# elador/FeatureDetection

Hardware: AMD Instinct MI355X
Metric: Mpatches/s (extract+WVM+SVM) per GPU, 640x480 pyramid (higher is better)
Workload: dtype u8/i32/f32/f64; 1 GPU; config 1/metric config: ffpDetectApp FaceFrontal.cfg five-stage cascade on 640x480 BGR frames: 13-layer pyramid, 20x20 windows step 1 (16185 windows/frame), HistEq64 -> WVM 280 filters -> OE -> RBF-SVM 1024 SV -> NMS; fd_pyramid_update_frames + fd_detect_five_stage_frames (the frames of a call share one pyramid aren...; frames_per_call=64, calls_in_flight=11, parallelism=image-shard dp1

## Files before the change

### featuredetection_amd/csrc/pyramid.hip

```cpp
#include "fd_internal.hpp"
#include <algorithm>
#include <cstring>

namespace {

constexpr int MAXJ = 16;

struct ResizeJob {
    int dw, dh;
    uint32_t dst_off;
    double scale_x, scale_y;
};
struct ResizeJobs {
    int n;
    ResizeJob j[MAXJ];
};
struct DownJob {
    int sw, sh;
    uint32_t src_off, dst_off;
};
struct FusedJob {
    int dw0, dh0, dw1, dh1;
    uint32_t dst0_off;
    uint32_t dst1_off;
    uint32_t xtab, ytab;
};
struct FusedJobs {
    int n;
    FusedJob j[MAXJ];
};
struct DownJobs {
    int n;
    int tile0[MAXJ + 1];
    DownJob j[MAXJ];
};
struct FilterJob {
    int w, h;
    uint32_t src_off, dst_off;
};
struct FilterJobs {
    int n;
    FilterJob j[MAXJ];
};

__device__ __forceinline__ int reflect101(int p, int len) {
    if (len == 1) return 0;
    while (p < 0 || p >= len) {
        if (p < 0) p = -p;
        else p = 2 * len - 2 - p;
    }
    return p;
}
__device__ __forceinline__ int reflect1(int p, int len) {
    if (len < 3) return reflect101(p, len);
    const int q = p < 0 ? -p : (p >= len ? 2 * len - 2 - p : p);
    return min(max(q, 0), len - 1);
}

struct FramePtrs {
    const uint8_t* p[FD_MAX_FRAMES];
};
__device__ __forceinline__ unsigned int mul24(unsigned int a, unsigned int b) {
    unsigned int r;
    asm("v_mul_u32_u24 %0, %1, %2" : "=v"(r) : "v"(a), "v"(b));
    return r;
}
__device__ __forceinline__ unsigned int mul24_s(unsigned int a_uniform, unsigned int b) {
    unsigned int r;
    asm("v_mul_u32_u24 %0, %1, %2" : "=v"(r) : "s"(a_uniform), "v"(b));
    return r;
}
__device__ __forceinline__ unsigned int mad24(unsigned int a, unsigned int b, unsigned int c) {
    unsigned int r;
    asm("v_mad_u32_u24 %0, %1, %2, %3" : "=v"(r) : "v"(a), "v"(b), "v"(c));
    return r;
}
__device__ __forceinline__ unsigned int mulhi24_s(unsigned int a_uniform, unsigned int b) {
    unsigned int r;
    asm("v_mul_hi_u32_u24 %0, %1, %2" : "=v"(r) : "s"(a_uniform), "v"(b));
    return r;
}
__device__ __forceinline__ uint32_t ld_u32_unaligned(const uint8_t* p) {
    uint32_t v;
    __builtin_memcpy(&v, p, 4);
    return v;
}
__device__ __forceinline__ uint32_t gray_of(uint32_t b, uint32_t g, uint32_t r) { return (b * 1868u + g * 9617u + r * 4899u + 8192u) >> 14; }

__global__ void k_frames_to_gray(FramePtrs frames, uint8_t* __restrict__ grayBase, size_t imageStride, int n, int ch) {
    const uint8_t* __restrict__ src = frames.p[blockIdx.y];
    uint8_t* __restrict__ gray = grayBase + (size_t)blockIdx.y * imageStride;
    const int nq = n >> 2;
    const bool aligned = ((uintptr_t)src & 3) == 0;
    const int stride = gridDim.x * blockDim.x;
    auto load3 = [&](int q, uint32_t (&w)[3]) {
        if (aligned) {
            const uint32_t* s3 = reinterpret_cast<const uint32_t*>(src) + 3 * (size_t)q;
            w[0] = s3[0]; w[1] = s3[1]; w[2] = s3[2];
        } else {
            const uint8_t* s1 = src + 12 * (size_t)q;
            w[0] = ld_u32_unaligned(s1); w[1] = ld_u32_unaligned(s1 + 4); w[2] = ld_u32_unaligned(s1 + 8);
        }
    };
    auto gray4 = [&](const uint32_t (&w)[3]) {
        const uint32_t g0 = gray_of(w[0] & 255u, (w[0] >> 8) & 255u, (w[0] >> 16) & 255u);
        const uint32_t g1 = gray_of(w[0] >> 24, w[1] & 255u, (w[1] >> 8) & 255u);
        const uint32_t g2 = gray_of((w[1] >> 16) & 255u, w[1] >> 24, w[2] & 255u);
        const uint32_t g3 = gray_of((w[2] >> 8) & 255u, (w[2] >> 16) & 255u, w[2] >> 24);
        return g0 | (g1 << 8) | (g2 << 16) | (g3 << 24);
    };
    constexpr int GQ = 4;
    for (int q = blockIdx.x * blockDim.x + threadIdx.x; q < nq; q += GQ * stride) {
        if (ch == 3) {
            uint32_t w[GQ][3];
// ... 157 lines not shown
        const int dx = dx0 + c;
        if (dx < jb.dw) {
            float fx;
            const int sx = srcX(dx, fx);
            const int a0 = __float2int_rn((1.f - fx) * 2048), a1 = __float2int_rn(fx * 2048);
            const int lx = sx - X0, lx1 = (sx + 1 < sw ? sx + 1 : sx) - X0;
            uint8_t* dp = dst + (uint32_t)((dy0 + rq * (TL_H / 4)) * jb.dw) + dx;
#pragma unroll
            for (int k = 0; k < TL_H / 4; ++k, dp += jb.dw) {
                const int rr = rq * (TL_H / 4) + k;
                if (dy0 + rr < jb.dh) {
                    const int4 rt = rowTab[rr];
                    const uint8_t* S0 = tile + rt.x;
                    const uint8_t* S1 = tile + rt.y;
                    const unsigned int r0 = __umul24(S0[lx], a0) + __umul24(S0[lx1], a1);
                    const unsigned int r1 = __umul24(S1[lx], a0) + __umul24(S1[lx1], a1);
                    *dp = (uint8_t)(((__umul24(rt.z, r0 >> 4) >> 16) + (__umul24(rt.w, r1 >> 4) >> 16) + 2) >> 2);
                }
            }
        }
        __syncthreads();
    }
}

#ifdef FD_PYR_PROF
constexpr int PYR_PROF_WGS = 65536;
__device__ unsigned long long fd_pyr_prof[PYR_PROF_WGS * 8];
#define PYR_T(x) const unsigned long long x = __builtin_amdgcn_s_memtime()
#else
#define PYR_T(x)
#endif
constexpr int FT_W1 = 62, FT_H1 = 16;
constexpr int G0_W = 2 * FT_W1 + 3, G0_H = 2 * FT_H1 + 3, G0_PITCH = 128;
constexpr int FS_PITCH = 256, FS_ROWS = 76;
constexpr int FS_LOADS = (FS_ROWS + 3) / 4;
struct FusedFetch {
    uint32_t v[FS_LOADS];
    int2 ex, ey;
};
__device__ __forceinline__ void fused_issue(FusedFetch& f, const uint8_t* __restrict__ src, int sw, const int2* __restrict__ tabs, const FusedJob& jb,
                                            const int4 d) {
    const int X0 = d.x & 0xffff, Y0 = (int)((uint32_t)d.x >> 16), ncol = d.y & 0xffff, nrow = (int)((uint32_t)d.y >> 16);
    const int gx0 = 2 * (d.z & 0xffff) * FT_W1 - 2;
    const int lane = threadIdx.x & 63, wave = __builtin_amdgcn_readfirstlane(threadIdx.x >> 6);
    const uint32_t voff = (uint32_t)(4 * min(lane, (ncol - 1) >> 2) + X0);
    const int rlast = nrow - 1;
#pragma unroll
    for (int q = 0; q < FS_LOADS; ++q) {
        const int r = min(wave + 4 * q, rlast);
        f.v[q] = ld_u32_unaligned(src + (uint32_t)((Y0 + r) * sw) + voff);
    }
    f.ex = tabs[jb.xtab + reflect101(gx0 + (int)(threadIdx.x & 127), jb.dw0)];
    {
        const int py = 2 * (int)((uint32_t)d.z >> 16) * FT_H1 - 2 + min(lane, G0_H - 1), pr = py < 0 ? -py : (py >= jb.dh0 ? 2 * jb.dh0 - 2 - py : py);
        f.ey = tabs[jb.ytab + min(max(pr, 0), jb.dh0 - 1)];
    }
}

__global__ __launch_bounds__(256) void k_resize_down(uint8_t* __restrict__ arena0, uint32_t src_off, int sw, int sh, const int2* __restrict__ tabs,
                                                     FusedJobs jobs, uint32_t tileTab, int tilesPerFrame, int nimg, size_t imageStride) {
    __shared__ __attribute__((aligned(16))) uint8_t stage[FS_ROWS * FS_PITCH];
    __shared__ __attribute__((aligned(16))) uint8_t g0[G0_H * G0_PITCH];
    const int4* tiles = reinterpret_cast<const int4*>(tabs + tileTab);
    const int lane = threadIdx.x & 63, wave = __builtin_amdgcn_readfirstlane(threadIdx.x >> 6);
    const bool byXcd = nimg >= 8 && (gridDim.x & 7u) == 0;
    const int xcd = blockIdx.x & 7;
    const int slot = byXcd ? (int)(blockIdx.x >> 3) : (int)blockIdx.x, nslot = byXcd ? (int)(gridDim.x >> 3) : (int)gridDim.x;
    const int items = (byXcd ? (nimg - xcd + 7) >> 3 : nimg) * tilesPerFrame;
    auto frame_of = [&](int item) { const int fi = item / tilesPerFrame; return byXcd ? xcd + 8 * fi : fi; };
    auto desc_of = [&](int item) { return item < items ? tiles[item % tilesPerFrame] : make_int4(0, 0, 0, 0); };

    int item = slot;
    if (item >= items) return;
    int4 d = desc_of(item);
    FusedFetch f;
    fused_issue(f, arena0 + (size_t)frame_of(item) * imageStride + src_off, sw, tabs, jobs.j[d.w], d);
    int itemN = item + nslot;
    int4 dN = desc_of(itemN);

#ifdef FD_PYR_PROF
    unsigned long long pacc[6] = {0, 0, 0, 0, 0, 0}, ptiles = 0;
#endif
    for (; item < items; item = itemN, d = dN, itemN += nslot, dN = desc_of(itemN)) {
        PYR_T(p0);
        const FusedJob jb = jobs.j[d.w];
        uint8_t* arena = arena0 + (size_t)frame_of(item) * imageStride;
        const int X0 = d.x & 0xffff, Y0 = (int)((uint32_t)d.x >> 16);
        const int x1 = (d.z & 0xffff) * FT_W1, y1 = (int)((uint32_t)d.z >> 16) * FT_H1;
        const int gx0 = 2 * x1 - 2, gy0 = 2 * y1 - 2;
        {
            static_assert(4 * (FS_LOADS - 1) + 3 < FS_ROWS && FS_PITCH == 256, "stage holds a dword per lane for rows wave + 4 q");
#pragma unroll
            for (int q = 0; q < FS_LOADS; ++q) *reinterpret_cast<uint32_t*>(&stage[(wave + 4 * q) * FS_PITCH + 4 * lane]) = f.v[q];
        }
        const int2 ex = f.ex, ey = f.ey;
        PYR_T(p1);
        __syncthreads();
        PYR_T(p2);
        if (itemN < items)
            fused_issue(f, arena0 + (size_t)frame_of(itemN) * imageStride + src_off, sw, tabs, jobs.j[dN.w], dN);
        PYR_T(p3);
        {
            const int c = threadIdx.x & 127, half = __builtin_amdgcn_readfirstlane(threadIdx.x >> 7);
            if (c < G0_W) {
                const uint8_t* sp = stage + (ex.x - X0);
                const unsigned int a0 = ex.y & 0xffff, a1 = (unsigned int)ex.y >> 16;
                uint8_t* gp = g0 + c;
                const unsigned int rowRec = (unsigned int)((ey.x & 0xffff) - Y0) | (((unsigned int)ey.y & 0xfffu) << 7) | ((((unsigned int)ey.y >> 16) & 0xfffu) << 19);
                const int rBase = half * (G0_H - 18);
#pragma unroll 2
                for (int i = 0; i < 18; i += 3) {
                    unsigned int s00[3], s01[3], s10[3], s11[3], b0s[3], b1s[3];
#pragma unroll
                    for (int q = 0; q < 3; ++q) {
                        const int r = rBase + i + q;
                        const unsigned int e = (unsigned int)__builtin_amdgcn_readlane((int)rowRec, r);
                        b0s[q] = ((e >> 7) & 0xfffu) << 12;
                        b1s[q] = (e >> 19) << 12;
                        const uint8_t* sr = sp + ((e & 127u) << 8);
                        s00[q] = sr[0]; s01[q] = sr[1]; s10[q] = sr[FS_PITCH]; s11[q] = sr[FS_PITCH + 1];
                    }
#pragma unroll
                    for (int q = 0; q < 3; ++q) {
                        const unsigned int h0 = mad24(s01[q], a1, mul24(s00[q], a0)) & ~15u;
                        const unsigned int h1 = mad24(s11[q], a1, mul24(s10[q], a0)) & ~15u;
                        const unsigned int v = (mulhi24_s(b0s[q], h0) + mulhi24_s(b1s[q], h1) + 2) >> 2;
                        gp[(rBase + i + q) * G0_PITCH] = (uint8_t)v;
                    }
                }
            }
        }
        PYR_T(p4);
        __syncthreads();
        PYR_T(p5);
        {
            const int c1 = lane;
            const int x = x1 + c1;
            if (c1 < FT_W1 && x < jb.dw1) {
                constexpr int PR = FT_H1 / 4;
                const uint8_t* T = g0 + (2 * wave * PR) * G0_PITCH + 2 * c1;
                int h[2 * PR + 3];
#pragma unroll
                for (int r = 0; r < 2 * PR + 3; ++r) {
                    const uint8_t* S = T + r * G0_PITCH;
                    const uint32_t p01 = *reinterpret_cast<const uint16_t*>(S), p23 = *reinterpret_cast<const uint16_t*>(S + 2);
                    h[r] = (int)__builtin_amdgcn_udot4(p01 | (p23 << 16), 0x04060401u, (uint32_t)S[4], false);
                }
                uint8_t* dp = arena + jb.dst1_off + (uint32_t)((y1 + wave * PR) * jb.dw1) + x;
#pragma unroll
                for (int j = 0; j < PR; ++j, dp += jb.dw1) {
                    if (y1 + wave * PR + j < jb.dh1) {
                        const int v = h[2 * j + 2] * 6 + (h[2 * j + 1] + h[2 * j + 3]) * 4 + h[2 * j] + h[2 * j + 4];
                        *dp = (uint8_t)((v + 128) >> 8);
                    }
                }
            }
        }
        if (jb.dst0_off != 0xffffffffu) {
            uint8_t* d0 = arena + jb.dst0_off;
            for (int i = threadIdx.x; i < 32 * 128; i += 256) {
                const int r = 2 + (i >> 7), c = 2 + (i & 127);
// ... 60 lines not shown
                        const uint8_t* row = src + (uint32_t)(reflect_cf(Y0 + r, sh) * sw);
                        uint32_t w = 0;
#pragma unroll
                        for (int b = 0; b < 4; ++b) w |= (uint32_t)row[reflect_cf(xs + b, sw)] << (8 * b);
                        v[k] = w;
                    }
                }
            }
#pragma unroll
            for (int k = 0; k < PD_LD; ++k) *reinterpret_cast<uint32_t*>(&tile[(2 * (rq + 4 * k) + half) * TL_PITCH + j4]) = v[k];
        }
        __syncthreads();
        const int x = dx0 + c;
        if (c < PD_W && x < dw) {
            constexpr int PR = PD_TH / 4;
            const uint8_t* T = tile + (2 * rq * PR) * TL_PITCH + 2 * c;
            int h[2 * PR + 3];
#pragma unroll
            for (int r = 0; r < 2 * PR + 3; ++r) {
                const uint8_t* S = T + r * TL_PITCH;
                const uint32_t p01 = *reinterpret_cast<const uint16_t*>(S), p23 = *reinterpret_cast<const uint16_t*>(S + 2);
                h[r] = (int)__builtin_amdgcn_udot4(p01 | (p23 << 16), 0x04060401u, (uint32_t)S[4], false);
            }
            uint8_t* dp = dst + (uint32_t)((dy0 + rq * PR) * dw) + x;
#pragma unroll
            for (int j = 0; j < PR; ++j, dp += dw) {
                if (dy0 + rq * PR + j < dh) {
                    const int v = h[2 * j + 2] * 6 + (h[2 * j + 1] + h[2 * j + 3]) * 4 + h[2 * j] + h[2 * j + 4];
                    *dp = (uint8_t)((v + 128) >> 8);
                }
            }
        }
        __syncthreads();
    }
}

__device__ __forceinline__ float grad_pair(const uint8_t* __restrict__ src, int w, int h, int x, int y, int ksize, int& gx, int& gy) {
    if (ksize == 1 || ksize == 3) {
        const int xm = reflect101(x - 1, w), xp = reflect101(x + 1, w);
        const int ym = reflect101(y - 1, h), yp = reflect101(y + 1, h);
        const uint8_t *S0 = src + (size_t)ym * w, *S1 = src + (size_t)y * w, *S2 = src + (size_t)yp * w;
        if (ksize == 1) {
            gx = S1[xp] - S1[xm];
            gy = S2[x] - S0[x];
            return 0.5f;
        }
        gx = (S0[xp] - S0[xm]) + 2 * (S1[xp] - S1[xm]) + (S2[xp] - S2[xm]);
        gy = (S2[xm] - S0[xm]) + 2 * (S2[x] - S0[x]) + (S2[xp] - S0[xp]);
        return 0.125f;
    }
    int a, d1, d2, d3, s0, s1, s2, s3;
    float scale;
    if (ksize == 5) { a = 2; d1 = 2; d2 = 1; d3 = 0; s0 = 6; s1 = 4; s2 = 1; s3 = 0; scale = 1.f / 128.f; }
    else if (ksize == 7) { a = 3; d1 = 5; d2 = 4; d3 = 1; s0 = 20; s1 = 15; s2 = 6; s3 = 1; scale = 1.f / 2048.f; }
    else { a = 1; d1 = 1; d2 = 0; d3 = 0; s0 = 10; s1 = 3; s2 = 0; s3 = 0; scale = 1.f / 32.f; }
    const int dk[4] = {0, d1, d2, d3}, sk[4] = {s0, s1, s2, s3};
    int cx[7], cy[7];
    for (int t = -a; t <= a; ++t) { cx[t + a] = reflect101(x + t, w); cy[t + a] = reflect101(y + t, h); }
    gx = 0;
    gy = 0;
    for (int j = -a; j <= a; ++j) {
        const uint8_t* S = src + (size_t)cy[j + a] * w;
        int rd = 0, rs = 0;
        for (int i = 1; i <= a; ++i) {
            const int hi = S[cx[a + i]], lo = S[cx[a - i]];
            rd += dk[i] * (hi - lo);
// ... 151 lines not shown
    lut.resize((size_t)65536 * E);
    for (int x = 0; x < 256; ++x) {
        double gradientX = ((double)x - 127) / 255;
        for (int y = 0; y < 256; ++y) {
            double gradientY = ((double)y - 127) / 255;
            double direction = std::atan2(gradientY, gradientX);
            double magnitude = std::sqrt(gradientX * gradientX + gradientY * gradientY);
            double bin;
            if (signedGradients) {
                direction += PI;
                bin = direction * bins / (2 * PI);
            } else {
                if (direction < 0) direction += PI;
                bin = direction * bins / PI;
            }
            auto sat = [](double v) { int r = fd_cvRound(v); return (uint8_t)(r < 0 ? 0 : (r > 255 ? 255 : r)); };
            size_t index = (size_t)x | ((size_t)y << 8);
            if (!interpolate) {
                lut[2 * index] = (uint8_t)((uint8_t)std::round(bin) % (unsigned)bins);
                lut[2 * index + 1] = sat(255 * magnitude);
            } else {
                uint8_t w1 = sat(255 * magnitude * (bin - std::floor(bin)));
                lut[4 * index] = (uint8_t)((uint8_t)std::floor(bin) % (unsigned)bins);
                lut[4 * index + 1] = sat(255 * magnitude - w1);
                lut[4 * index + 2] = (uint8_t)((uint8_t)std::ceil(bin) % (unsigned)bins);
                lut[4 * index + 3] = w1;
            }
        }
    }
}

void build_resize_tables(fd_pyramid* p, int W, int H) {
    p->rtab_x.assign(p->all.size(), ~0u);
    p->rtab_y.assign(p->all.size(), ~0u);
    static const int mode = [] { const char* e = getenv("FD_PYR_FUSED"); return e ? atoi(e) : 1; }();
    if (mode == 0) return;
    std::vector<int2> tab;
    std::vector<std::vector<int4>> tiles;
    p->rtile_off.clear();
    p->rtile_cnt.clear();
    int nfused = 0;
    for (size_t k = 0; k + 1 < p->all.size(); ++k) {
        const HostLayer& L = p->all[k];
        const HostLayer& D = p->all[k + 1];
        if (L.depth != 0 || D.depth != 1 || D.chain != L.chain) continue;
        if (L.w == W && L.h == H && L.gray_off == p->gray_full_off) continue;
        if (L.w < 3 || L.h < 3 || W > 65535 || H > 65535) continue;
        if (L.kept && mode != 2) continue;
        const double scale_x = 1. / ((double)L.w / W), scale_y = 1. / ((double)L.h / H);
        std::vector<int2> xt((size_t)L.w), yt((size_t)L.h);
        for (int dx = 0; dx < L.w; ++dx) {
            float fx = (float)((dx + 0.5) * scale_x - 0.5);
            int sx = (int)floorf(fx);
            fx -= sx;
            if (sx < 0) { fx = 0; sx = 0; }
            if (sx >= W - 1) { fx = 0; sx = W - 1; }
            const int a0 = (int)nearbyintf((1.f - fx) * 2048), a1 = (int)nearbyintf(fx * 2048);
            xt[(size_t)dx] = make_int2(sx, a0 | (a1 << 16));
        }
        for (int dy = 0; dy < L.h; ++dy) {
            float fy = (float)((dy + 0.5) * scale_y - 0.5);
            const int sy = (int)floorf(fy);
            fy -= sy;
            const int b0 = (int)nearbyintf((1.f - fy) * 2048), b1 = (int)nearbyintf(fy * 2048);
            const int y0 = sy < 0 ? 0 : (sy >= H ? H - 1 : sy), y1 = sy + 1 < 0 ? 0 : (sy + 1 >= H ? H - 1 : sy + 1);
            yt[(size_t)dy] = make_int2(y0 | (y1 << 16), b0 | (b1 << 16));
        }
        bool fits = true;
        for (int dy = 0; dy < L.h && fits; ++dy) {
            const int y0 = yt[(size_t)dy].x & 0xffff, y1 = (int)((uint32_t)yt[(size_t)dy].x >> 16), b0 = yt[(size_t)dy].y & 0xffff, b1 = (int)((uint32_t)yt[(size_t)dy].y >> 16);
            fits = (y1 == y0 + 1 || b1 == 0) && b0 >= 0 && b0 <= 2048 && b1 >= 0 && b1 <= 2048 && y1 >= y0;
        }
        for (int x1 = 0; x1 < D.w && fits; x1 += FT_W1) {
            const int cLo = std::max(0, 2 * x1 - 2), cHi = std::min(L.w - 1, 2 * x1 - 2 + G0_W - 1);
            fits = std::min(W - 1, xt[(size_t)cHi].x + 1) - xt[(size_t)cLo].x + 1 <= FS_PITCH;
        }
        for (int y1 = 0; y1 < D.h && fits; y1 += FT_H1) {
            const int rLo = std::max(0, 2 * y1 - 2), rHi = std::min(L.h - 1, 2 * y1 - 2 + G0_H - 1);
            fits = (yt[(size_t)rHi].x >> 16) - (yt[(size_t)rLo].x & 0xffff) + 1 <= FS_ROWS;
        }
        if (!fits) continue;
        {
            if (nfused % MAXJ == 0) tiles.emplace_back();
            std::vector<int4>& tl = tiles.back();
            for (int ty = 0; ty * FT_H1 < D.h; ++ty)
                for (int tx = 0; tx * FT_W1 < D.w; ++tx) {
                    const int gx0 = 2 * tx * FT_W1 - 2, gy0 = 2 * ty * FT_H1 - 2;
                    const int cLo = std::max(0, gx0), cHi = std::min(L.w - 1, gx0 + G0_W - 1), rLo = std::max(0, gy0), rHi = std::min(L.h - 1, gy0 + G0_H - 1);
                    const int X0 = xt[(size_t)cLo].x, Y0 = yt[(size_t)rLo].x & 0xffff;
                    const int ncol = std::min(W - 1, xt[(size_t)cHi].x + 1) - X0 + 1, nrow = (yt[(size_t)rHi].x >> 16) - Y0 + 1;
                    tl.push_back(make_int4((int)((uint32_t)X0 | (uint32_t)Y0 << 16), (int)((uint32_t)ncol | (uint32_t)nrow << 16),
                                           (int)((uint32_t)tx | (uint32_t)ty << 16), nfused % MAXJ));
                }
            ++nfused;
        }
        p->rtab_x[k] = (uint32_t)tab.size();
        tab.insert(tab.end(), xt.begin(), xt.end());
        p->rtab_y[k] = (uint32_t)tab.size();
        tab.insert(tab.end(), yt.begin(), yt.end());
    }
    if (tab.empty()) return;
    for (const std::vector<int4>& tl : tiles) {
        if (tab.size() & 1) tab.push_back(make_int2(0, 0));
        p->rtile_off.push_back((uint32_t)tab.size());
        p->rtile_cnt.push_back((int)tl.size());
        for (const int4& t : tl) { tab.push_back(make_int2(t.x, t.y)); tab.push_back(make_int2(t.z, t.w)); }
    }
    p->rtab.reserve(sizeof(int2) * tab.size());
    HIP_CHECK(hipMemcpy(p->rtab.p, tab.data(), sizeof(int2) * tab.size(), hipMemcpyHostToDevice));
}

void build_layout(fd_pyramid* p, int W, int H) {
    p->img_w = W;
    p->img_h = H;
    p->all.clear();
    p->kept.clear();
    size_t off = 0;
    p->gray_full_off = 0;
    off = align256((size_t)W * H);
    const int fch = p->filter_kind == FD_LAYER_GRADBIN ? (p->interpolate ? 4 : 2) : 1;
    for (size_t i = 0; i < p->octl; ++i) {
        double scaleFactor = std::pow(p->inc, (double)i);
        int w = fd_cvRound(W * scaleFactor), h = fd_cvRound(H * scaleFactor);
        if (w < 1 || h < 1) FD_THROW(FD_ERR_INVALID_ARGUMENT, "ImagePyramid: layer %zu would be empty", i);
        int depth = 0;
        const bool isFull = (w == W && h == H);
        HostLayer L{(int)i, scaleFactor, w, h, 1, (uint32_t)(isFull ? p->gray_full_off : off), 0, scaleFactor <= p->maxS && scaleFactor >= p->minS, (int)i, depth};
        if (!isFull) off = align256(off + (size_t)w * h);
        p->all.push_back(L);
        int pw = w, ph = h;
        scaleFactor *= 0.5;
        for (size_t j = 1; scaleFactor >= p->minS && pw > 1; ++j, scaleFactor *= 0.5) {
// ... 22 lines not shown
    }
    if (off > 0xfffffff0ull) FD_THROW(FD_ERR_INVALID_ARGUMENT, "ImagePyramid: pyramid exceeds 4 GB arena");
    std::sort(p->kept.begin(), p->kept.end(), [&](int a, int b) { return p->all[a].index < p->all[b].index; });
    p->arena_bytes = off + 256;
    p->image_stride = (p->arena_bytes + 255) & ~(size_t)255;
    if (p->nimg > 1 && p->image_stride * (size_t)p->nimg > 0xfffffff0ull * 16) FD_THROW(FD_ERR_INVALID_ARGUMENT, "ImagePyramid: multi-frame pyramid too large");
    p->arena.reserve(p->image_stride * (size_t)p->nimg);
    p->h_layer_table.clear();
    for (int k : p->kept) {
        const HostLayer& L = p->all[k];
        p->h_layer_table.push_back(LayerDesc{L.w, L.h, L.ch, 0, L.gray_off, L.filt_off});
    }
    p->layer_table.reserve(sizeof(LayerDesc) * std::max<size_t>(1, p->h_layer_table.size()));
    if (!p->h_layer_table.empty())
        HIP_CHECK(hipMemcpyAsync(p->layer_table.p, p->h_layer_table.data(), sizeof(LayerDesc) * p->h_layer_table.size(),
                                 hipMemcpyHostToDevice, p->ctx->stream));
    build_resize_tables(p, W, H);
}

int grid_for(int npix) { return std::max(1, std::min(1024, (npix + 255) / 256)); }
int tile_grid_for(int ntiles) { return std::max(1, std::min(1024, ntiles)); }

void pyramid_update(fd_pyramid* p, const uint8_t* image, int W, int H, int ch, int is_device, hipStream_t st, const uint8_t* const* frames = nullptr) {
    if (!image && !frames) FD_THROW(FD_ERR_INVALID_ARGUMENT, "fd_pyramid_update: image is NULL");
    if (p->nimg > 1 && !frames) FD_THROW(FD_ERR_INVALID_ARGUMENT, "fd_pyramid_update: the pyramid holds %d frames, use fd_pyramid_update_frames", p->nimg);
    if (p->nimg > 1 && p->filter_kind != FD_LAYER_NONE) FD_THROW(FD_ERR_INVALID_ARGUMENT, "multi-frame pyramids have no layer filters");
    if (W < 1 || H < 1) FD_THROW(FD_ERR_INVALID_ARGUMENT, "fd_pyramid_update: empty image");
    if (ch != 1 && ch != 3) FD_THROW(FD_ERR_INVALID_ARGUMENT, "fd_pyramid_update: image must have 1 or 3 channels");
    if (W != p->img_w || H != p->img_h || p->all.empty()) build_layout(p, W, H);
    uint8_t* arena = p->arena.as<uint8_t>();
    const size_t npix = (size_t)W * H;
    const int NI = frames ? p->nimg : 1;
    const size_t IS = p->image_stride;
    auto enqueue_rest = [&]() {
    int maxDepth = 0;
    for (const HostLayer& L : p->all) maxDepth = std::max(maxDepth, L.depth);
    {
        ResizeJobs jobs;
        jobs.n = 0;
        int maxpix = 0, maxtiles = 0;
        auto flush = [&]() {
            if (!jobs.n) return;
            bool fits = true;
            for (int q = 0; q < jobs.n; ++q)
                fits = fits && jobs.j[q].scale_x >= 1.0 && jobs.j[q].scale_x <= 2.05 && jobs.j[q].scale_y >= 1.0 && jobs.j[q].scale_y <= 2.05;
            if (fits)
                hipLaunchKernelGGL(k_resize_tiled, dim3(tile_grid_for(maxtiles), jobs.n, NI), dim3(256), 0, st, arena, arena, p->gray_full_off, W, H, jobs, IS);
            else
                hipLaunchKernelGGL(k_resize_linear, dim3(grid_for(maxpix), jobs.n, NI), dim3(256), 0, st, arena, arena, p->gray_full_off, W, H, jobs, IS);
            jobs.n = 0;
            maxpix = 0;
            maxtiles = 0;
        };
        for (size_t k = 0; k < p->all.size(); ++k) {
            const HostLayer& L = p->all[k];
            if (L.depth != 0) continue;
            if (L.w == W && L.h == H && L.gray_off == p->gray_full_off) continue;
            if (p->rtab_x[k] != ~0u) continue;
            ResizeJob& j = jobs.j[jobs.n++];
            j.dw = L.w; j.dh = L.h; j.dst_off = L.gray_off;
            j.scale_x = 1. / ((double)L.w / W);
            j.scale_y = 1. / ((double)L.h / H);
            maxpix = std::max(maxpix, L.w * L.h);
            maxtiles = std::max(maxtiles, ((L.w + TL_W - 1) / TL_W) * ((L.h + TL_H - 1) / TL_H));
            if (jobs.n == MAXJ) flush();
        }
        flush();
    }
    {
        FusedJobs jobs;
        jobs.n = 0;
        size_t group = 0;
        auto flush = [&]() {
            if (!jobs.n) return;
            static int perCu = 0;
            if (perCu == 0 && (hipOccupancyMaxActiveBlocksPerMultiprocessor(&perCu, k_resize_down, 256, 0) != hipSuccess || perCu < 1)) perCu = 4;
            const int tilesPerFrame = p->rtile_cnt[group];
            int grid = (int)std::min<int64_t>((int64_t)tilesPerFrame * NI, (int64_t)p->ctx->num_cus * perCu);
            if (NI >= 8 && grid >= 64) grid &= ~7;
            hipLaunchKernelGGL(k_resize_down, dim3(grid), dim3(256), 0, st, arena, p->gray_full_off, W, H, p->rtab.as<int2>(), jobs, p->rtile_off[group], tilesPerFrame, NI, IS);
            jobs.n = 0;
            ++group;
        };
        for (size_t k = 0; k + 1 < p->all.size(); ++k) {
            if (p->rtab_x[k] == ~0u) continue;
            const HostLayer& L = p->all[k];
            const HostLayer& D = p->all[k + 1];
            FusedJob& j = jobs.j[jobs.n++];
            j.dw0 = L.w; j.dh0 = L.h; j.dw1 = D.w; j.dh1 = D.h;
            j.dst0_off = (L.kept && L.gray_off != p->gray_full_off) ? L.gray_off : 0xffffffffu;
            j.dst1_off = D.gray_off;
            j.xtab = p->rtab_x[k]; j.ytab = p->rtab_y[k];
            if (jobs.n == MAXJ) flush();
        }
        flush();
    }
    {
        DownJobs dj;
        dj.n = 0;
        dj.tile0[0] = 0;
        auto flush1 = [&]() {
            if (!dj.n) return;
            hipLaunchKernelGGL(k_pyrdown_tiled, dim3(tile_grid_for(dj.tile0[dj.n]), 1, NI), dim3(256), 0, st, arena, dj, IS);
            dj.n = 0;
        };
        for (size_t k = 1; k < p->all.size(); ++k) {
            const HostLayer& L = p->all[k];
            if (L.depth != 1 || p->rtab_x[k - 1] != ~0u) continue;
            const HostLayer& S = p->all[k - 1];
            DownJob& j = dj.j[dj.n++];
            j.sw = S.w; j.sh = S.h; j.src_off = S.gray_off; j.dst_off = L.gray_off;
            dj.tile0[dj.n] = dj.tile0[dj.n - 1] + ((L.w + PD_W - 1) / PD_W) * ((L.h + PD_TH - 1) / PD_TH);
            if (dj.n == MAXJ) flush1();
        }
        flush1();
    }
    for (int d = 2; d <= maxDepth; ++d) {
        DownJobs jobs;
        jobs.n = 0;
        jobs.tile0[0] = 0;
        auto flush = [&]() {
            if (!jobs.n) return;
            hipLaunchKernelGGL(k_pyrdown_tiled, dim3(tile_grid_for(jobs.tile0[jobs.n]), 1, NI), dim3(256), 0, st, arena, jobs, IS);
            jobs.n = 0;
        };
        for (size_t k = 0; k < p->all.size(); ++k) {
            const HostLayer& L = p->all[k];
            if (L.depth != d) continue;
            const HostLayer& S = p->all[k - 1];
            DownJob& j = jobs.j[jobs.n++];
            j.sw = S.w; j.sh = S.h; j.src_off = S.gray_off; j.dst_off = L.gray_off;
            jobs.tile0[jobs.n] = jobs.tile0[jobs.n - 1] + ((L.w + PD_W - 1) / PD_W) * ((L.h + PD_TH - 1) / PD_TH);
            if (jobs.n == MAXJ) flush();
        }
        flush();
    }
    if (p->filter_kind != FD_LAYER_NONE) {
        FilterJobs jobs, bjobs;
        jobs.n = 0;
        bjobs.n = 0;
        int maxpix = 0;
// ... 9 lines not shown
                else
                    hipLaunchKernelGGL(k_gradbin<2>, g, dim3(256), 0, st, arena, p->lut.as<uint8_t>(), p->grad_kernel, jobs);
            } else {
                hipLaunchKernelGGL(k_lbp, g, dim3(256), 0, st, arena, p->lbp_type, jobs);
            }
            jobs.n = 0;
            maxpix = 0;
        };
        for (int k : p->kept) {
            const HostLayer& L = p->all[k];
            FilterJob& j = jobs.j[jobs.n++];
            j.w = L.w; j.h = L.h; j.src_off = blur ? L.blur_off : L.gray_off; j.dst_off = L.filt_off;
            if (blur) {
                FilterJob& b = bjobs.j[bjobs.n++];
                b.w = L.w; b.h = L.h; b.src_off = L.gray_off; b.dst_off = L.blur_off;
            }
            maxpix = std::max(maxpix, L.w * L.h);
            if (jobs.n == MAXJ) flush();
        }
        flush();
    }
    };
    if (frames) {
        FramePtrs fp;
        if (!is_device) {
            p->input.reserve(npix * ch * (size_t)NI);
            for (int f = 0; f < NI; ++f) {
                HIP_CHECK(hipMemcpyAsync(p->input.as<uint8_t>() + (size_t)f * npix * ch, frames[f], npix * ch, hipMemcpyHostToDevice, st));
                fp.p[f] = p->input.as<uint8_t>() + (size_t)f * npix * ch;
            }
        } else {
            for (int f = 0; f < NI; ++f) fp.p[f] = frames[f];
        }
        hipLaunchKernelGGL(k_frames_to_gray, dim3(grid_for((int)(npix / 16 + 1)), NI), dim3(256), 0, st, fp, arena + p->gray_full_off, IS, (int)npix, ch);
    } else {
        const uint8_t* dimg = image;
        if (!is_device) {
            p->input.reserve(npix * ch);
            HIP_CHECK(hipMemcpyAsync(p->input.p, image, npix * ch, hipMemcpyHostToDevice, st));
            dimg = p->input.as<uint8_t>();
        }
        if (ch == 3) {
            hipLaunchKernelGGL(k_bgr2gray, dim3(grid_for((int)npix)), dim3(256), 0, st, dimg, arena + p->gray_full_off, (int)npix);
        } else {
            HIP_CHECK(hipMemcpyAsync(arena + p->gray_full_off, dimg, npix, hipMemcpyDeviceToDevice, st));
        }
    }
    enqueue_rest();
    HIP_CHECK(hipGetLastError());
    if (!p->ready) HIP_CHECK(hipEventCreateWithFlags(&p->ready, hipEventDisableTiming));
    HIP_CHECK(hipEventRecord(p->ready, st));
    p->readyStream = st;
    p->version++;
}

}

void fd_pyramid_update_on(fd_pyramid* p, const uint8_t* image, int w, int h, int ch, int is_device, hipStream_t st) {
    if (!p) FD_THROW(FD_ERR_INVALID_ARGUMENT, "fd_pyramid_update: NULL pyramid");
    HIP_CHECK(hipSetDevice(p->ctx->device));
    pyramid_update(p, image, w, h, ch, is_device, st);
}

void fd_enumerate_layers(const fd_pyramid* p, int pw, int ph, int sx, int sy, const int* roiIn,
                         std::vector<WindowLayer>& out, int64_t& total) {
    if (sx < 1) FD_THROW(FD_ERR_INVALID_ARGUMENT, "DirectPyramidFeatureExtractor: stepX has to be greater than zero");
    if (sy < 1) FD_THROW(FD_ERR_INVALID_ARGUMENT, "DirectPyramidFeatureExtractor: stepY has to be greater than zero");
// ... 356 lines not shown
```

### featuredetection_amd/csrc/fd_internal.hpp

```cpp
#pragma once
#include <hip/hip_runtime.h>
#include <cstdint>
#include <cstdio>
#include <cstdlib>
#include <cmath>
#include <map>
#include <memory>
#include <string>
#include <typeindex>
#include <typeinfo>
#include <vector>
#include <stdexcept>
#include <atomic>
#include <condition_variable>
#include <functional>
#include <mutex>
#include <thread>
#include <deque>
#include <exception>
#include "../../include/fd_hip.h"
#include "../../include/fd_hip_bench.h"

struct FdPinned {
    void* p = nullptr;
// ... 282 lines not shown
};

struct HostLayer {
    int index;
    double scale;
    int w, h, ch;
    uint32_t gray_off, filt_off;
    bool kept;
    int chain, depth;
    uint32_t blur_off = 0;
};

struct WindowLayer {
    int32_t layer;
    int32_t bx, by;
    int32_t nx, ny;
    int32_t ow, oh;
    int64_t first;
};

struct fd_pyramid {
    fd_ctx* ctx;
    size_t octl;
    double inc, minS, maxS;
    int filter_kind = FD_LAYER_NONE, bins = 9, signed_gradients = 0, interpolate = 0, grad_kernel = 1, lbp_type = 0;
    int grad_blur = 0;
    int img_w = 0, img_h = 0;
    std::vector<HostLayer> all;
    std::vector<int> kept;
    DevBuf arena;
    DevBuf input;
    DevBuf lut;
    DevBuf rtab;
    std::vector<uint32_t> rtab_x, rtab_y;
    std::vector<uint32_t> rtile_off;
    std::vector<int> rtile_cnt;
    DevBuf layer_table;
    std::vector<LayerDesc> h_layer_table;
    uint32_t gray_full_off = 0;
    size_t arena_bytes = 0;
    uint64_t version = 0;
    int nimg = 1;
    size_t image_stride = 0;
    int sel_first = -1, sel_last = -1, sel_step = 1;
    int view_first = -1, view_last = -1;
    bool sel_has_roi = false;
    int sel_roi[4] = {0, 0, 0, 0};
    hipEvent_t ready = nullptr;
    hipStream_t readyStream = nullptr;
    ~fd_pyramid() { if (ready) (void)hipEventDestroy(ready); }
};

static inline void fd_pyramid_require_single(const fd_pyramid* p, const char* who) {
    if (p->nimg > 1) FD_THROW(FD_ERR_INVALID_ARGUMENT, "%s: the pyramid holds %d frames (fd_pyramid_set_frames); use fd_detect_five_stage_frames", who, p->nimg);
}

static inline void fd_pyramid_wait(const fd_pyramid* p, hipStream_t consumer) {
    if (p->ready && consumer != p->readyStream) HIP_CHECK(hipStreamWaitEvent(consumer, p->ready, 0));
}

void fd_pyramid_update_on(fd_pyramid* p, const uint8_t* image, int w, int h, int ch, int is_device, hipStream_t st);
constexpr int FD_MAX_FRAMES = 64;
void fd_enumerate_layers(const fd_pyramid* p, int pw, int ph, int sx, int sy, const int* roi,
                         std::vector<WindowLayer>& out, int64_t& total);

void fd_host_overlap_elimination(const fd_detection* in, int n, float dist, float ratio, std::vector<int>& keep);
void fd_host_block_nms_sparse(const std::vector<fd_detection>& pos, int imgW, int imgH, int sz, bool masked,
// ... 2 lines not shown
```

Baseline: 3707 Mpatches/s.

## Fuse BGR-to-gray conversion with the first pyramid downsample for multi-frame input

Adds a kernel that loads BGR frame tiles, converts them to gray, writes the full-resolution gray image and computes the first 2x pyrDown level from shared memory in the same pass. This removes a separate downsample launch and the re-read of the full gray image. Reflect borders are handled inside the tile. The path is on by default, can be disabled with an environment variable, and uses frame-interleaved block ordering when the frame count is a multiple of eight. It also masks a row index in the resize kernel.

```diff
diff --git a/featuredetection_amd/csrc/pyramid.hip b/featuredetection_amd/csrc/pyramid.hip
--- a/featuredetection_amd/csrc/pyramid.hip
+++ b/featuredetection_amd/csrc/pyramid.hip
@@ -377,7 +377,7 @@
                 const uint8_t* sp = stage + (ex.x - X0);
                 const unsigned int a0 = ex.y & 0xffff, a1 = (unsigned int)ex.y >> 16;
                 uint8_t* gp = g0 + c;
-                const unsigned int rowRec = (unsigned int)((ey.x & 0xffff) - Y0) | (((unsigned int)ey.y & 0xfffu) << 7) | ((((unsigned int)ey.y >> 16) & 0xfffu) << 19);
+                const unsigned int rowRec = ((unsigned int)((ey.x & 0xffff) - Y0) & 127u) | (((unsigned int)ey.y & 0xfffu) << 7) | ((((unsigned int)ey.y >> 16) & 0xfffu) << 19);
                 const int rBase = half * (G0_H - 18);
 #pragma unroll 2
                 for (int i = 0; i < 18; i += 3) {
@@ -524,6 +524,111 @@
             }
         }
         __syncthreads();
+    }
+}
+
+constexpr int GD_QUADS = 33, GD_ROWS = 2 * PD_TH + 3, GD_PITCH = 4 * GD_QUADS + 4;
+constexpr int GD_ITEMS = (GD_QUADS * GD_ROWS + 255) / 256;
+template <int CH>
+__global__ __launch_bounds__(256) void k_frames_gray_down(FramePtrs frames, uint8_t* __restrict__ arena0, size_t imageStride, uint32_t grayOff,
+                                                          uint32_t dstOff, int W, int H, int tilesX, int tilesPerFrame, int nimg) {
+    __shared__ __attribute__((aligned(16))) uint8_t tile[GD_ROWS * GD_PITCH];
+    int frame, t;
+    if ((nimg & 7) == 0) {
+        const int slot = (int)(blockIdx.x >> 3);
+        frame = (int)(blockIdx.x & 7) + 8 * (slot / tilesPerFrame);
+        t = slot % tilesPerFrame;
+    } else {
+        frame = (int)blockIdx.x / tilesPerFrame;
+        t = (int)blockIdx.x - frame * tilesPerFrame;
+    }
+    const uint8_t* __restrict__ src = frames.p[frame];
+    uint8_t* __restrict__ arena = arena0 + (size_t)frame * imageStride;
+    uint8_t* __restrict__ gray = arena + grayOff;
+    const int dw = W >> 1, dh = (H + 1) >> 1;
+    const int ty = t / tilesX, tx = t - ty * tilesX;
+    const int x1 = tx * PD_W, y1 = ty * PD_TH;
+    const int Q0 = 31 * tx - 1, Y0 = 2 * y1 - 2;
+    const int nq = W >> 2;
+    uint32_t gv[GD_ITEMS];
+    int gofs[GD_ITEMS];
+    {
+        uint32_t w[GD_ITEMS][CH];
+        int qq[GD_ITEMS], rr[GD_ITEMS];
+#pragma unroll
+        for (int k = 0; k < GD_ITEMS; ++k) {
+            const int i = min((int)threadIdx.x + 256 * k, GD_QUADS * GD_ROWS - 1);
+            const int r = i / GD_QUADS, q = i - r * GD_QUADS;
+            qq[k] = q;
+            rr[k] = r;
+            const int gq = min(max(Q0 + q, 0), nq - 1);
+            const uint32_t* s = reinterpret_cast<const uint32_t*>(src + (uint32_t)(reflect_cf(Y0 + r, H) * W + 4 * gq) * CH);
+#pragma unroll
+            for (int c = 0; c < CH; ++c) w[k][c] = s[c];
+        }
+        __builtin_amdgcn_sched_barrier(0);
+#pragma unroll
+        for (int k = 0; k < GD_ITEMS; ++k) {
+            uint32_t g;
+            if constexpr (CH == 3) {
+                const uint32_t* v = w[k];
+                const uint32_t g0 = gray_of(v[0] & 255u, (v[0] >> 8) & 255u, (v[0] >> 16) & 255u);
+                const uint32_t g1 = gray_of(v[0] >> 24, v[1] & 255u, (v[1] >> 8) & 255u);
+                const uint32_t g2 = gray_of((v[1] >> 16) & 255u, v[1] >> 24, v[2] & 255u);
+                const uint32_t g3 = gray_of((v[2] >> 8) & 255u, (v[2] >> 16) & 255u, v[2] >> 24);
+                g = g0 | (g1 << 8) | (g2 << 16) | (g3 << 24);
+            } else {
+                g = w[k][0];
+            }
+            const int q = qq[k], r = rr[k];
+            const bool item = (int)threadIdx.x + 256 * k < GD_QUADS * GD_ROWS;
+            if (item) *reinterpret_cast<uint32_t*>(&tile[r * GD_PITCH + 4 * q]) = g;
+            const int gq = Q0 + q, gy = Y0 + r;
+            gv[k] = g;
+            gofs[k] = item && q >= 1 && q <= 31 && r >= 2 && r <= 33 && gq < nq && gy < H ? gy * W + 4 * gq : -1;
+        }
+    }
+    __syncthreads();
+    if (tx == 0 || 4 * (Q0 + GD_QUADS) > W) {
+        const int gx0 = 4 * Q0;
+        uint8_t v = 0;
+        int dcol = -1;
+        if (threadIdx.x < 4 * GD_ROWS) {
+            const int r = threadIdx.x >> 2, j = threadIdx.x & 3;
+            const int x = j < 2 ? -2 + j : W + (j - 2);
+            const int xs = j < 2 ? -x : 2 * W - 2 - x;
+            if (x - gx0 >= 0 && x - gx0 < 4 * GD_QUADS && xs - gx0 >= 0 && xs - gx0 < 4 * GD_QUADS) {
+                v = tile[r * GD_PITCH + xs - gx0];
+                dcol = r * GD_PITCH + x - gx0;
+            }
+        }
+        __syncthreads();
+        if (dcol >= 0) tile[dcol] = v;
+        __syncthreads();
+    }
+#pragma unroll
+    for (int k = 0; k < GD_ITEMS; ++k)
+        if (gofs[k] >= 0) *reinterpret_cast<uint32_t*>(gray + (uint32_t)gofs[k]) = gv[k];
+    const int c = threadIdx.x & 63, rq = __builtin_amdgcn_readfirstlane(threadIdx.x >> 6);
+    const int x = x1 + c;
+    if (c < PD_W && x < dw) {
+        constexpr int PR = PD_TH / 4;
+        const uint8_t* T = tile + (2 * rq * PR) * GD_PITCH + 2 * c + 2;
+        int h[2 * PR + 3];
+#pragma unroll
+        for (int r = 0; r < 2 * PR + 3; ++r) {
+            const uint8_t* S = T + r * GD_PITCH;
+            const uint32_t p01 = *reinterpret_cast<const uint16_t*>(S), p23 = *reinterpret_cast<const uint16_t*>(S + 2);
+            h[r] = (int)__builtin_amdgcn_udot4(p01 | (p23 << 16), 0x04060401u, (uint32_t)S[4], false);
+        }
+        uint8_t* dp = arena + dstOff + (uint32_t)((y1 + rq * PR) * dw) + x;
+#pragma unroll
+        for (int j = 0; j < PR; ++j, dp += dw) {
+            if (y1 + rq * PR + j < dh) {
+                const int v = h[2 * j + 2] * 6 + (h[2 * j + 1] + h[2 * j + 3]) * 4 + h[2 * j] + h[2 * j + 4];
+                *dp = (uint8_t)((v + 128) >> 8);
+            }
+        }
     }
 }
 
@@ -895,6 +1000,9 @@
     const size_t npix = (size_t)W * H;
     const int NI = frames ? p->nimg : 1;
     const size_t IS = p->image_stride;
+    int grayDownK = -1;
+    const char* gdEnv = getenv("FD_PYR_GRAY_DOWN");
+    const bool grayDown = frames && !(gdEnv && atoi(gdEnv) <= 0);
     auto enqueue_rest = [&]() {
     int maxDepth = 0;
     for (const HostLayer& L : p->all) maxDepth = std::max(maxDepth, L.depth);
@@ -969,7 +1077,7 @@
         };
         for (size_t k = 1; k < p->all.size(); ++k) {
             const HostLayer& L = p->all[k];
-            if (L.depth != 1 || p->rtab_x[k - 1] != ~0u) continue;
+            if (L.depth != 1 || p->rtab_x[k - 1] != ~0u || (int)k == grayDownK) continue;
             const HostLayer& S = p->all[k - 1];
             DownJob& j = dj.j[dj.n++];
             j.sw = S.w; j.sh = S.h; j.src_off = S.gray_off; j.dst_off = L.gray_off;
@@ -1045,7 +1153,22 @@
         } else {
             for (int f = 0; f < NI; ++f) fp.p[f] = frames[f];
         }
-        hipLaunchKernelGGL(k_frames_to_gray, dim3(grid_for((int)(npix / 16 + 1)), NI), dim3(256), 0, st, fp, arena + p->gray_full_off, IS, (int)npix, ch);
+        bool gd = grayDown && W % 4 == 0 && W >= 8 && H >= 3 && npix * ch < (size_t)INT32_MAX;
+        for (int f = 0; f < NI && gd; ++f) gd = ((uintptr_t)fp.p[f] & 3) == 0;
+        for (size_t k = 1; k < p->all.size() && gd; ++k) {
+            const HostLayer& S = p->all[k - 1];
+            if (p->all[k].depth == 1 && S.w == W && S.h == H && S.gray_off == p->gray_full_off && p->rtab_x[k - 1] == ~0u) grayDownK = (int)k;
+        }
+        if (grayDownK >= 0) {
+            const HostLayer& D = p->all[grayDownK];
+            const int tilesX = (D.w + PD_W - 1) / PD_W, tiles = tilesX * ((D.h + PD_TH - 1) / PD_TH);
+            if (ch == 3)
+                hipLaunchKernelGGL(k_frames_gray_down<3>, dim3(tiles * NI), dim3(256), 0, st, fp, arena, IS, p->gray_full_off, D.gray_off, W, H, tilesX, tiles, NI);
+            else
+                hipLaunchKernelGGL(k_frames_gray_down<1>, dim3(tiles * NI), dim3(256), 0, st, fp, arena, IS, p->gray_full_off, D.gray_off, W, H, tilesX, tiles, NI);
+        } else {
+            hipLaunchKernelGGL(k_frames_to_gray, dim3(grid_for((int)(npix / 16 + 1)), NI), dim3(256), 0, st, fp, arena + p->gray_full_off, IS, (int)npix, ch);
+        }
     } else {
         const uint8_t* dimg = image;
         if (!is_device) {
```

After: 3707 Mpatches/s (median of 4 runs). Within noise of the previous version (+0.0%).

## Stage per-row source pairs in fused resize and compute vertical taps on device

Applied to the files above, without the earlier changes.

The fused resize+pyrdown kernel no longer stages a contiguous band of source rows described by a precomputed y-table. Each wave lane now computes its own vertical source row and bilinear weights from scale_y, then loads the two source rows each output row needs into stage slots. The per-row weights go through a small shared taps array, and the horizontal interpolation uses packed udot2. This removes the y-table gather, the readlane row decode and the row-span fit check, which lets layers whose row span exceeded the stage still take the fused path. In exchange the kernel does extra float math per tile and uses a different staging layout, and device-side float rounding must match the old host-computed table.

```diff
diff --git a/featuredetection_amd/csrc/fd_internal.hpp b/featuredetection_amd/csrc/fd_internal.hpp
--- a/featuredetection_amd/csrc/fd_internal.hpp
+++ b/featuredetection_amd/csrc/fd_internal.hpp
@@ -338,7 +338,7 @@
     DevBuf input;
     DevBuf lut;
     DevBuf rtab;
-    std::vector<uint32_t> rtab_x, rtab_y;
+    std::vector<uint32_t> rtab_x;
     std::vector<uint32_t> rtile_off;
     std::vector<int> rtile_cnt;
     DevBuf layer_table;
diff --git a/featuredetection_amd/csrc/pyramid.hip b/featuredetection_amd/csrc/pyramid.hip
--- a/featuredetection_amd/csrc/pyramid.hip
+++ b/featuredetection_amd/csrc/pyramid.hip
@@ -23,7 +23,8 @@
     int dw0, dh0, dw1, dh1;
     uint32_t dst0_off;
     uint32_t dst1_off;
-    uint32_t xtab, ytab;
+    uint32_t xtab;
+    double scale_y;
 };
 struct FusedJobs {
     int n;
@@ -75,11 +76,12 @@
     asm("v_mad_u32_u24 %0, %1, %2, %3" : "=v"(r) : "v"(a), "v"(b), "v"(c));
     return r;
 }
-__device__ __forceinline__ unsigned int mulhi24_s(unsigned int a_uniform, unsigned int b) {
+__device__ __forceinline__ unsigned int mulhi24(unsigned int a, unsigned int b) {
     unsigned int r;
-    asm("v_mul_hi_u32_u24 %0, %1, %2" : "=v"(r) : "s"(a_uniform), "v"(b));
+    asm("v_mul_hi_u32_u24 %0, %1, %2" : "=v"(r) : "v"(a), "v"(b));
     return r;
 }
+typedef unsigned short u16x2 __attribute__((ext_vector_type(2)));
 __device__ __forceinline__ uint32_t ld_u32_unaligned(const uint8_t* p) {
     uint32_t v;
     __builtin_memcpy(&v, p, 4);
@@ -303,35 +305,38 @@
 #endif
 constexpr int FT_W1 = 62, FT_H1 = 16;
 constexpr int G0_W = 2 * FT_W1 + 3, G0_H = 2 * FT_H1 + 3, G0_PITCH = 128;
-constexpr int FS_PITCH = 256, FS_ROWS = 76;
-constexpr int FS_LOADS = (FS_ROWS + 3) / 4;
+constexpr int FS_PITCH = 256;
+constexpr int FS_LOADS = (2 * G0_H + 3) / 4;
 struct FusedFetch {
     uint32_t v[FS_LOADS];
-    int2 ex, ey;
+    int2 ex;
+    uint32_t taps;
 };
-__device__ __forceinline__ void fused_issue(FusedFetch& f, const uint8_t* __restrict__ src, int sw, const int2* __restrict__ tabs, const FusedJob& jb,
-                                            const int4 d) {
-    const int X0 = d.x & 0xffff, Y0 = (int)((uint32_t)d.x >> 16), ncol = d.y & 0xffff, nrow = (int)((uint32_t)d.y >> 16);
-    const int gx0 = 2 * (d.z & 0xffff) * FT_W1 - 2;
+__device__ __forceinline__ void fused_issue(FusedFetch& f, const uint8_t* __restrict__ src, int sw, int sh, const int2* __restrict__ tabs,
+                                            const FusedJob& jb, const int4 d) {
+    const int X0 = d.x, ncol = d.y;
+    const int gx0 = 2 * (d.z & 0xffff) * FT_W1 - 2, gy0 = 2 * (int)((uint32_t)d.z >> 16) * FT_H1 - 2;
     const int lane = threadIdx.x & 63, wave = __builtin_amdgcn_readfirstlane(threadIdx.x >> 6);
+    uint32_t rowOff;
+    {
+        const int py = gy0 + min((wave >> 1) + 2 * lane, G0_H - 1), pr = py < 0 ? -py : (py >= jb.dh0 ? 2 * jb.dh0 - 2 - py : py);
+        float fy = (float)((min(max(pr, 0), jb.dh0 - 1) + 0.5) * jb.scale_y - 0.5);
+        const int sy = (int)floorf(fy);
+        fy -= sy;
+        f.taps = (uint32_t)__float2int_rn((1.f - fy) * 2048) | (uint32_t)__float2int_rn(fy * 2048) << 16;
+        rowOff = mul24((uint32_t)min(max(sy + (wave & 1), 0), sh - 1), (uint32_t)sw);
+    }
     const uint32_t voff = (uint32_t)(4 * min(lane, (ncol - 1) >> 2) + X0);
-    const int rlast = nrow - 1;
-#pragma unroll
-    for (int q = 0; q < FS_LOADS; ++q) {
-        const int r = min(wave + 4 * q, rlast);
-        f.v[q] = ld_u32_unaligned(src + (uint32_t)((Y0 + r) * sw) + voff);
-    }
+#pragma unroll
+    for (int q = 0; q < FS_LOADS; ++q) f.v[q] = ld_u32_unaligned(src + ((uint32_t)__builtin_amdgcn_readlane((int)rowOff, q) + voff));
     f.ex = tabs[jb.xtab + reflect101(gx0 + (int)(threadIdx.x & 127), jb.dw0)];
-    {
-        const int py = 2 * (int)((uint32_t)d.z >> 16) * FT_H1 - 2 + min(lane, G0_H - 1), pr = py < 0 ? -py : (py >= jb.dh0 ? 2 * jb.dh0 - 2 - py : py);
-        f.ey = tabs[jb.ytab + min(max(pr, 0), jb.dh0 - 1)];
-    }
 }
 
 __global__ __launch_bounds__(256) void k_resize_down(uint8_t* __restrict__ arena0, uint32_t src_off, int sw, int sh, const int2* __restrict__ tabs,
                                                      FusedJobs jobs, uint32_t tileTab, int tilesPerFrame, int nimg, size_t imageStride) {
-    __shared__ __attribute__((aligned(16))) uint8_t stage[FS_ROWS * FS_PITCH];
+    __shared__ __attribute__((aligned(16))) uint8_t stage[4 * FS_LOADS * FS_PITCH];
     __shared__ __attribute__((aligned(16))) uint8_t g0[G0_H * G0_PITCH];
+    __shared__ uint2 taps[G0_H];
     const int4* tiles = reinterpret_cast<const int4*>(tabs + tileTab);
     const int lane = threadIdx.x & 63, wave = __builtin_amdgcn_readfirstlane(threadIdx.x >> 6);
     const bool byXcd = nimg >= 8 && (gridDim.x & 7u) == 0;
@@ -345,7 +350,7 @@
     if (item >= items) return;
     int4 d = desc_of(item);
     FusedFetch f;
-    fused_issue(f, arena0 + (size_t)frame_of(item) * imageStride + src_off, sw, tabs, jobs.j[d.w], d);
+    fused_issue(f, arena0 + (size_t)frame_of(item) * imageStride + src_off, sw, sh, tabs, jobs.j[d.w], d);
     int itemN = item + nslot;
     int4 dN = desc_of(itemN);
 
@@ -356,48 +361,42 @@
         PYR_T(p0);
         const FusedJob jb = jobs.j[d.w];
         uint8_t* arena = arena0 + (size_t)frame_of(item) * imageStride;
-        const int X0 = d.x & 0xffff, Y0 = (int)((uint32_t)d.x >> 16);
+        const int X0 = d.x;
         const int x1 = (d.z & 0xffff) * FT_W1, y1 = (int)((uint32_t)d.z >> 16) * FT_H1;
         const int gx0 = 2 * x1 - 2, gy0 = 2 * y1 - 2;
         {
-            static_assert(4 * (FS_LOADS - 1) + 3 < FS_ROWS && FS_PITCH == 256, "stage holds a dword per lane for rows wave + 4 q");
+            static_assert(2 * G0_H <= 4 * FS_LOADS && FS_PITCH == 256, "stage holds a dword per lane for slots wave + 4 q");
 #pragma unroll
             for (int q = 0; q < FS_LOADS; ++q) *reinterpret_cast<uint32_t*>(&stage[(wave + 4 * q) * FS_PITCH + 4 * lane]) = f.v[q];
-        }
-        const int2 ex = f.ex, ey = f.ey;
+            const int i = (wave >> 1) + 2 * lane;
+            if ((wave & 1) == 0 && i < G0_H) taps[i] = make_uint2((f.taps & 0xffffu) << 12, (f.taps >> 16) << 12);
+        }
+        const int2 ex = f.ex;
         PYR_T(p1);
         __syncthreads();
         PYR_T(p2);
         if (itemN < items)
-            fused_issue(f, arena0 + (size_t)frame_of(itemN) * imageStride + src_off, sw, tabs, jobs.j[dN.w], dN);
+            fused_issue(f, arena0 + (size_t)frame_of(itemN) * imageStride + src_off, sw, sh, tabs, jobs.j[dN.w], dN);
         PYR_T(p3);
         {
             const int c = threadIdx.x & 127, half = __builtin_amdgcn_readfirstlane(threadIdx.x >> 7);
             if (c < G0_W) {
-                const uint8_t* sp = stage + (ex.x - X0);
-                const unsigned int a0 = ex.y & 0xffff, a1 = (unsigned int)ex.y >> 16;
-                uint8_t* gp = g0 + c;
-                const unsigned int rowRec = (unsigned int)((ey.x & 0xffff) - Y0) | (((unsigned int)ey.y & 0xfffu) << 7) | ((((unsigned int)ey.y >> 16) & 0xfffu) << 19);
                 const int rBase = half * (G0_H - 18);
-#pragma unroll 2
-                for (int i = 0; i < 18; i += 3) {
-                    unsigned int s00[3], s01[3], s10[3], s11[3], b0s[3], b1s[3];
-#pragma unroll
-                    for (int q = 0; q < 3; ++q) {
-                        const int r = rBase + i + q;
-                        const unsigned int e = (unsigned int)__builtin_amdgcn_readlane((int)rowRec, r);
-                        b0s[q] = ((e >> 7) & 0xfffu) << 12;
-                        b1s[q] = (e >> 19) << 12;
-                        const uint8_t* sr = sp + ((e & 127u) << 8);
-                        s00[q] = sr[0]; s01[q] = sr[1]; s10[q] = sr[FS_PITCH]; s11[q] = sr[FS_PITCH + 1];
-                    }
-#pragma unroll
-                    for (int q = 0; q < 3; ++q) {
-                        const unsigned int h0 = mad24(s01[q], a1, mul24(s00[q], a0)) & ~15u;
-                        const unsigned int h1 = mad24(s11[q], a1, mul24(s10[q], a0)) & ~15u;
-                        const unsigned int v = (mulhi24_s(b0s[q], h0) + mulhi24_s(b1s[q], h1) + 2) >> 2;
-                        gp[(rBase + i + q) * G0_PITCH] = (uint8_t)v;
-                    }
+                const int lx = min(max(ex.x - X0, 0), FS_PITCH - 1) + 2 * rBase * FS_PITCH;
+                int lx1 = lx + 1;
+                asm("" : "+v"(lx1));
+                const uint8_t *sp = stage + lx, *sp1 = stage + lx1;
+                const uint2* tp = taps + rBase;
+                const u16x2 aw = __builtin_bit_cast(u16x2, ex.y);
+                uint8_t* gp = g0 + rBase * G0_PITCH + c;
+#pragma unroll
+                for (int i = 0; i < 18; ++i) {
+                    const uint8_t *s = sp + 2 * i * FS_PITCH, *s1 = sp1 + 2 * i * FS_PITCH;
+                    const u16x2 p0 = {s[0], s1[0]}, p1 = {s[FS_PITCH], s1[FS_PITCH]};
+                    const uint2 t = tp[i];
+                    const unsigned int h0 = __builtin_amdgcn_udot2(p0, aw, 0u, false) & ~15u;
+                    const unsigned int h1 = __builtin_amdgcn_udot2(p1, aw, 0u, false) & ~15u;
+                    gp[i * G0_PITCH] = (uint8_t)((mulhi24(t.x, h0) + mulhi24(t.y, h1) + 2) >> 2);
                 }
             }
         }
@@ -741,7 +740,6 @@
 
 void build_resize_tables(fd_pyramid* p, int W, int H) {
     p->rtab_x.assign(p->all.size(), ~0u);
-    p->rtab_y.assign(p->all.size(), ~0u);
     static const int mode = [] { const char* e = getenv("FD_PYR_FUSED"); return e ? atoi(e) : 1; }();
     if (mode == 0) return;
     std::vector<int2> tab;
@@ -756,8 +754,8 @@
         if (L.w == W && L.h == H && L.gray_off == p->gray_full_off) continue;
         if (L.w < 3 || L.h < 3 || W > 65535 || H > 65535) continue;
         if (L.kept && mode != 2) continue;
-        const double scale_x = 1. / ((double)L.w / W), scale_y = 1. / ((double)L.h / H);
-        std::vector<int2> xt((size_t)L.w), yt((size_t)L.h);
+        const double scale_x = 1. / ((double)L.w / W);
+        std::vector<int2> xt((size_t)L.w);
         for (int dx = 0; dx < L.w; ++dx) {
             float fx = (float)((dx + 0.5) * scale_x - 0.5);
             int sx = (int)floorf(fx);
@@ -767,26 +765,10 @@
             const int a0 = (int)nearbyintf((1.f - fx) * 2048), a1 = (int)nearbyintf(fx * 2048);
             xt[(size_t)dx] = make_int2(sx, a0 | (a1 << 16));
         }
-        for (int dy = 0; dy < L.h; ++dy) {
-            float fy = (float)((dy + 0.5) * scale_y - 0.5);
-            const int sy = (int)floorf(fy);
-            fy -= sy;
-            const int b0 = (int)nearbyintf((1.f - fy) * 2048), b1 = (int)nearbyintf(fy * 2048);
-            const int y0 = sy < 0 ? 0 : (sy >= H ? H - 1 : sy), y1 = sy + 1 < 0 ? 0 : (sy + 1 >= H ? H - 1 : sy + 1);
-            yt[(size_t)dy] = make_int2(y0 | (y1 << 16), b0 | (b1 << 16));
-        }
         bool fits = true;
-        for (int dy = 0; dy < L.h && fits; ++dy) {
-            const int y0 = yt[(size_t)dy].x & 0xffff, y1 = (int)((uint32_t)yt[(size_t)dy].x >> 16), b0 = yt[(size_t)dy].y & 0xffff, b1 = (int)((uint32_t)yt[(size_t)dy].y >> 16);
-            fits = (y1 == y0 + 1 || b1 == 0) && b0 >= 0 && b0 <= 2048 && b1 >= 0 && b1 <= 2048 && y1 >= y0;
-        }
         for (int x1 = 0; x1 < D.w && fits; x1 += FT_W1) {
             const int cLo = std::max(0, 2 * x1 - 2), cHi = std::min(L.w - 1, 2 * x1 - 2 + G0_W - 1);
             fits = std::min(W - 1, xt[(size_t)cHi].x + 1) - xt[(size_t)cLo].x + 1 <= FS_PITCH;
-        }
-        for (int y1 = 0; y1 < D.h && fits; y1 += FT_H1) {
-            const int rLo = std::max(0, 2 * y1 - 2), rHi = std::min(L.h - 1, 2 * y1 - 2 + G0_H - 1);
-            fits = (yt[(size_t)rHi].x >> 16) - (yt[(size_t)rLo].x & 0xffff) + 1 <= FS_ROWS;
         }
         if (!fits) continue;
         {
@@ -794,19 +776,15 @@
             std::vector<int4>& tl = tiles.back();
             for (int ty = 0; ty * FT_H1 < D.h; ++ty)
                 for (int tx = 0; tx * FT_W1 < D.w; ++tx) {
-                    const int gx0 = 2 * tx * FT_W1 - 2, gy0 = 2 * ty * FT_H1 - 2;
-                    const int cLo = std::max(0, gx0), cHi = std::min(L.w - 1, gx0 + G0_W - 1), rLo = std::max(0, gy0), rHi = std::min(L.h - 1, gy0 + G0_H - 1);
-                    const int X0 = xt[(size_t)cLo].x, Y0 = yt[(size_t)rLo].x & 0xffff;
-                    const int ncol = std::min(W - 1, xt[(size_t)cHi].x + 1) - X0 + 1, nrow = (yt[(size_t)rHi].x >> 16) - Y0 + 1;
-                    tl.push_back(make_int4((int)((uint32_t)X0 | (uint32_t)Y0 << 16), (int)((uint32_t)ncol | (uint32_t)nrow << 16),
-                                           (int)((uint32_t)tx | (uint32_t)ty << 16), nfused % MAXJ));
+                    const int gx0 = 2 * tx * FT_W1 - 2;
+                    const int cLo = std::max(0, gx0), cHi = std::min(L.w - 1, gx0 + G0_W - 1);
+                    const int X0 = xt[(size_t)cLo].x, ncol = std::min(W - 1, xt[(size_t)cHi].x + 1) - X0 + 1;
+                    tl.push_back(make_int4(X0, ncol, (int)((uint32_t)tx | (uint32_t)ty << 16), nfused % MAXJ));
                 }
             ++nfused;
         }
         p->rtab_x[k] = (uint32_t)tab.size();
         tab.insert(tab.end(), xt.begin(), xt.end());
-        p->rtab_y[k] = (uint32_t)tab.size();
-        tab.insert(tab.end(), yt.begin(), yt.end());
     }
     if (tab.empty()) return;
     for (const std::vector<int4>& tl : tiles) {
@@ -953,7 +931,8 @@
             j.dw0 = L.w; j.dh0 = L.h; j.dw1 = D.w; j.dh1 = D.h;
             j.dst0_off = (L.kept && L.gray_off != p->gray_full_off) ? L.gray_off : 0xffffffffu;
             j.dst1_off = D.gray_off;
-            j.xtab = p->rtab_x[k]; j.ytab = p->rtab_y[k];
+            j.xtab = p->rtab_x[k];
+            j.scale_y = 1. / ((double)L.h / H);
             if (jobs.n == MAXJ) flush();
         }
         flush();
```

Measured after the change: 3663 Mpatches/s before, 3763 Mpatches/s after, median of 6. 2.7% higher.
